# ltiao/bore

Hardware: NVIDIA B200
Metric: mlp_value_and_input_grad_evals_per_sec (higher is better)
Workload: dtype f32 MLP / f64 L-BFGS-B

## Files before the change

### bore_b200/csrc/lbfgsb.cu

```cuda
#include <float.h>
#include <math.h>
#include <stdlib.h>
#include <string.h>

#include <algorithm>
#include <cmath>

#include "common.cuh"
#include "lbfgsb_fused.h"
#include "lbfgsb_types.h"

namespace lbw {
#define LB_VARIANT 1
#include "lbfgsb_core.h"
#undef LB_VARIANT
}
namespace lbw10 {
#define LB_VARIANT 1
#define LB_MCONST 10
#include "lbfgsb_core.h"
#undef LB_MCONST
#undef LB_VARIANT
}

template <int MC> struct LbCore;
template <> struct LbCore<0> {
  using Work = lbw::LbWork;
  static __device__ __forceinline__ void carve(Work &w, double *d, int *i, int n, int m) { lbw::lb_carve(w, d, i, n, m); }
  template <class Mem>
  static __device__ __forceinline__ int advance(const LbParams &P, Work &w, LbScal &s, Mem &mem, int stage) {
    return lbw::lb_advance(P, w, s, mem, stage);
  }
};
template <> struct LbCore<10> {
  using Work = lbw10::LbWork;
  static __device__ __forceinline__ void carve(Work &w, double *d, int *i, int n, int m) { lbw10::lb_carve(w, d, i, n, m); }
  template <class Mem>
  static __device__ __forceinline__ int advance(const LbParams &P, Work &w, LbScal &s, Mem &mem, int stage) {
    return lbw10::lb_advance(P, w, s, mem, stage);
  }
};
namespace {

constexpr int SCAL_BYTES = LB_SCAL_DOUBLES * sizeof(double);
static_assert(sizeof(LbScal) <= SCAL_BYTES, "LbScal grew past its slot");

struct LbLayout {
  size_t lo, hi, nbd, cnt, work, evals, lists, xf, f, g, pend, blocks, block_stride, total;
};

__host__ __device__ inline size_t align_up(size_t a, size_t b) { return (a + b - 1) / b * b; }

inline LbLayout make_layout(int S, int n, int m) {
  LbLayout L;
  size_t o = 0;
  L.lo = o; o += align_up(n * sizeof(double), 16);
  L.hi = o; o += align_up(n * sizeof(double), 16);
  L.nbd = o; o += align_up(n * sizeof(int), 16);
  L.cnt = o; o += 16;
  L.work = o; o += 16;
  L.evals = o; o += 16;
  L.lists = o; o += align_up((size_t)2 * S * sizeof(int), 16);
  L.xf = o; o += align_up((size_t)S * n * sizeof(float), 16);
  L.f = o; o += align_up((size_t)S * sizeof(float), 16);
  L.g = o; o += align_up((size_t)S * n * sizeof(float), 16);
  L.pend = o; o += align_up((size_t)S * sizeof(int), 16);
  o = align_up(o, 256);
  L.block_stride = align_up((size_t)LB_PERSIST_DOUBLES(n, m) * sizeof(double), 128);
  L.blocks = o; o += L.block_stride * S;
  L.total = o;
  return L;
}

struct LbDev {
  LbParams P;
  int S;
  char *blocks;
  size_t block_stride;
  double *xreq;
  float *xf;
  const void *F;
  const void *G;
  int *lists;
  int *cnt;
  int *work;
  unsigned long long *evals;
  unsigned long long *bytes;
  int *pend;
};

__device__ __forceinline__ LbScal *scal_of(const LbDev &D, int sid) {
  return reinterpret_cast<LbScal *>(D.blocks + D.block_stride * sid);
}

__device__ __forceinline__ unsigned long long step_bytes(int n, int fg_size, bool was_ls,
                                                         bool heavy, int col_in, int col_out,
                                                         bool pend, bool updated) {
  unsigned long long b = 2ull * sizeof(LbScal) + (unsigned long long)fg_size * (1 + n) + 8ull * n;
  if (was_ls) b += 32ull * n;
  if (heavy && col_in > 0) b += 16ull * n * col_in + 32ull * col_in * col_in;
  b += pend ? 12ull * n : 8ull * n;
  if (heavy && pend) b += 32ull * n;
  if (updated) b += 16ull * n + 48ull * col_out + 8ull * col_out * col_out;
  return b;
}

__global__ void __launch_bounds__(128) lbfgsb_init_kernel(LbDev D, const double *__restrict__ X0) {
  const int n = D.P.n;
  const int warp = (blockIdx.x * blockDim.x + threadIdx.x) >> 5;
  const int nwarps = (gridDim.x * blockDim.x) >> 5;
  const int lane = threadIdx.x & 31;
  if (blockIdx.x == 0 && threadIdx.x == 0) {
    D.cnt[0] = D.S; D.cnt[1] = 0; D.cnt[2] = 0;
    D.work[0] = 0; D.work[1] = 0; D.work[2] = 0;
    *D.evals = 0ULL;
    *D.bytes = 0ULL;
  }
  for (int sid = warp; sid < D.S; sid += nwarps) {
    for (int i = lane; i < n; i += 32) {
      double xi = X0[(size_t)sid * n + i];
      const int nb = D.P.nbd[i];
      if (nb > 0) {
        if (nb <= 2 && xi <= D.P.lo[i]) xi = D.P.lo[i];
        else if (nb >= 2 && xi >= D.P.hi[i]) xi = D.P.hi[i];
      }
      D.xreq[(size_t)sid * n + i] = xi;
      if (D.xf) D.xf[(size_t)sid * n + i] = (float)xi;
    }
    if (lane == 0) {
      LbScal s;
      s.f = 0; s.fold = 0; s.theta = 1.0; s.gd = 0; s.gdold = 0; s.dtd = 0; s.dnorm = 0;
      s.stp = 0; s.stpmx = 0; s.sbgnrm = 0;
      s.finit = s.ginit = s.gtest = s.gx = s.gy = s.fx = s.fy = 0;
      s.stx = s.sty = s.stmin = s.stmax = s.width = s.width1 = 0;
      s.phase = LB_PH_START; s.col = 0; s.iupdat = 0; s.iter = 0; s.nit = 0;
      s.nfev = 1;
      s.ifun = 0; s.iback = 0; s.updatd = 0; s.status = -1; s.task = 0;
      s.brackt = 0; s.stage = 0; s.ls_task = LB_LS_START; s.nskip = 0; s.nintol = 0;
      s.resume = 0;
      *scal_of(D, sid) = s;
      D.lists[sid] = sid;
      if (D.pend) D.pend[sid] = 1;
    }
  }
}

__device__ __forceinline__ uint32_t smem_u32(const void *p) {
  return (uint32_t)__cvta_generic_to_shared(p);
}
__device__ __forceinline__ void mbar_init(uint64_t *bar, int count) {
  asm volatile("mbarrier.init.shared::cta.b64 [%0], %1;" ::"r"(smem_u32(bar)), "r"(count) : "memory");
}
__device__ __forceinline__ void mbar_expect_tx(uint64_t *bar, uint32_t bytes) {
  asm volatile("mbarrier.arrive.expect_tx.shared::cta.b64 _, [%0], %1;" ::"r"(smem_u32(bar)), "r"(bytes)
               : "memory");
}
__device__ __forceinline__ void mbar_wait(uint64_t *bar, uint32_t parity) {
  asm volatile(
      "{\n"
      ".reg .pred p;\n"
      "LB_WAIT:\n"
      "mbarrier.try_wait.parity.shared::cta.b64 p, [%0], %1;\n"
      "@p bra LB_DONE;\n"
      "bra LB_WAIT;\n"
      "LB_DONE:\n"
      "}\n" ::"r"(smem_u32(bar)), "r"(parity)
      : "memory");
}
__device__ __forceinline__ void bulk_g2s(void *dst_smem, const void *src, uint32_t bytes, uint64_t *bar) {
  asm volatile("cp.async.bulk.shared::cluster.global.mbarrier::complete_tx::bytes [%0], [%1], %2, [%3];"
               ::"r"(smem_u32(dst_smem)), "l"(src), "r"(bytes), "r"(smem_u32(bar))
               : "memory");
}
__device__ __forceinline__ void bulk_s2g(void *dst, const void *src_smem, uint32_t bytes) {
  asm volatile("cp.async.bulk.global.shared::cta.bulk_group [%0], [%1], %2;" ::"l"(dst),
               "r"(smem_u32(src_smem)), "r"(bytes)
               : "memory");
}
__device__ __forceinline__ void bulk_commit() { asm volatile("cp.async.bulk.commit_group;" ::: "memory"); }
__device__ __forceinline__ void bulk_wait_read() {
  asm volatile("cp.async.bulk.wait_group.read 0;" ::: "memory");
}
__device__ __forceinline__ void bulk_wait_all() {
  asm volatile("cp.async.bulk.wait_group 0;" ::: "memory");
}
__device__ __forceinline__ void bulk_prefetch_l2(const void *src, uint32_t bytes) {
  asm volatile("cp.async.bulk.prefetch.L2.global [%0], %1;" ::"l"(src), "r"(bytes) : "memory");
}
__device__ __forceinline__ void fence_async_smem() {
  asm volatile("fence.proxy.async.shared::cta;" ::: "memory");
}

constexpr int LB_NPHASE_MAX = 4;

struct BlockMem {
  bool loaded = false, is_dirty = false, vec_dirty = false, requested = false;
  __device__ bool ld_kept() { return false; }
  int nph = 0, cap = LB_NPHASE_MAX;
  uint64_t *bar = nullptr;
  uint32_t parity = 0;
  __device__ void load() {
    if (!loaded && requested) { mbar_wait(bar, parity); __syncwarp(); }
    loaded = true;
  }
  __device__ void dirty() { is_dirty = true; }
  __device__ void dirty_vec() { vec_dirty = true; }
  __device__ void phase() {
    if (nph < cap) { __syncthreads(); ++nph; }
  }
};

__host__ __device__ inline size_t lb_header_bytes(int n, int wpb) {
  return align_up(LB_FORMK_ACC * 32 * sizeof(int), 16) + 2 * align_up(n * sizeof(double), 16) +
         align_up(n * sizeof(int), 16) + align_up(2 * wpb * sizeof(uint64_t) + 2 * sizeof(int), 16);
}

template <typename FG, int MC>
__global__ void __maxnreg__(168) lbfgsb_warp_kernel(LbDev D, int round, size_t warp_bytes, int nphase, int kofn, int pf) {
  extern __shared__ __align__(128) unsigned char smem_raw[];
  const int n = D.P.n, m = D.P.m;
  const int wib = threadIdx.x >> 5, lane = threadIdx.x & 31;
  const int wpb = blockDim.x >> 5;
  const int cur = round % 3, nxt = (round + 1) % 3, clr = (round + 2) % 3;
  if (blockIdx.x == 0 && threadIdx.x == 0) { D.cnt[clr] = 0; D.work[clr] = 0; }
  const int n_active = D.cnt[cur];
  if (blockIdx.x * wpb >= n_active) return;
  const int *list_cur = D.lists + (size_t)(round & 1) * D.S;
  int *list_nxt = D.lists + (size_t)((round + 1) & 1) * D.S;
  int *qhead = D.work + cur;

  int *ftab = reinterpret_cast<int *>(smem_raw);
  double *s_lo = reinterpret_cast<double *>(smem_raw + align_up(LB_FORMK_ACC * 32 * sizeof(int), 16));
  double *s_hi = s_lo + align_up(n * sizeof(double), 16) / sizeof(double);
  int *s_nbd = reinterpret_cast<int *>(s_hi + align_up(n * sizeof(double), 16) / sizeof(double));
  uint64_t *bars = reinterpret_cast<uint64_t *>(reinterpret_cast<unsigned char *>(s_nbd) +
                                                align_up(n * sizeof(int), 16));
  uint64_t *bar = bars + 2 * wib, *bar2 = bar + 1;
  unsigned char *base = smem_raw + lb_header_bytes(n, wpb) + warp_bytes * wib;
  const uint32_t block_bytes = (uint32_t)(LB_PERSIST_DOUBLES(n, m) * sizeof(double));
  const uint32_t p1_bytes = (uint32_t)(SCAL_BYTES + 4 * LB_NV(n) * sizeof(double));
  const uint32_t p2_bytes = block_bytes - p1_bytes;

  int &kn_wait = reinterpret_cast<int *>(bars + 2 * wpb)[0];
  int &kn_done = reinterpret_cast<int *>(bars + 2 * wpb)[1];
  if (threadIdx.x == 0) { kn_wait = 0; kn_done = 0; }
  auto claim = [&]() {
    int v = 0;
    if (lane == 0) v = atomicAdd(qhead, 1);
    return __shfl_sync(0xffffffffu, v, 0);
  };
  int cur_i = claim();
  int nxt_sid = -1;
  if (lane == 0) {
    mbar_init(bar, 1);
    mbar_init(bar2, 1);
    asm volatile("fence.mbarrier_init.release.cluster;" ::: "memory");
    if (cur_i < n_active) {
      mbar_expect_tx(bar, p1_bytes);
      bulk_g2s(base, D.blocks + D.block_stride * list_cur[cur_i], p1_bytes, bar);
    }
  }
  int nxt_i = n_active;
#pragma unroll 1
  for (int o = threadIdx.x; o < LB_FORMK_ACC * 32; o += blockDim.x) ftab[o] = lbw::lb_formk_code(o, m);
#pragma unroll 1
  for (int i = threadIdx.x; i < n; i += blockDim.x) {
    s_lo[i] = D.P.lo[i];
    s_hi[i] = D.P.hi[i];
    s_nbd[i] = D.P.nbd[i];
  }
  __syncthreads();
  LbParams P = D.P;
  P.lo = s_lo; P.hi = s_hi; P.nbd = s_nbd;

  typename LbCore<MC>::Work w;
  LbCore<MC>::carve(w, reinterpret_cast<double *>(base),
                    reinterpret_cast<int *>(base + lbw::lb_work_doubles(n, m) * sizeof(double)), n, m);
  w.ftab = ftab;
  LbScal *s_smem = reinterpret_cast<LbScal *>(base);
  const FG *F = static_cast<const FG *>(D.F);
  const FG *G = static_cast<const FG *>(D.G);
  uint32_t parity = 0, parity2 = 0;
  unsigned long long my_bytes = 0, my_evals = 0;

  LbScal s;
  BlockMem mem;
  int sid = 0, col_in = 0;
  bool was_ls = false;

  auto finish = [&](int pend) {
    char *gblock = D.blocks + D.block_stride * sid;
    double *xr = D.xreq + (size_t)sid * n;
    if (mem.requested) {
      if (!mem.loaded) mbar_wait(bar2, parity2);
      parity2 ^= 1;
    }
    __syncwarp();
    my_bytes += step_bytes(n, (int)sizeof(FG), was_ls, mem.loaded, col_in, s.col, pend != 0, mem.is_dirty);
    if (pend) {
      int changed = 0;
      float *xf = D.xf ? D.xf + (size_t)sid * n : nullptr;
#pragma unroll 1
      for (int i = lane; i < n; i += 32) {
        const double xi = w.x[i];
        changed |= (xr[i] != xi);
        xr[i] = xi;
        if (xf) xf[i] = (float)xi;
      }
      if (__any_sync(0xffffffffu, changed)) s.nfev += 1;
    } else {
#pragma unroll 1
      for (int i = lane; i < n; i += 32) xr[i] = w.x[i];
    }
    if (lane == 0) *s_smem = s;
    fence_async_smem();
    __syncwarp();
    cur_i = nxt_i;
    if (lane == 0) {
      uint32_t bytes = SCAL_BYTES;
      if (pend && mem.vec_dirty) bytes += 4 * LB_NV(n) * sizeof(double);
      if (pend && mem.is_dirty) bytes = block_bytes;
      bulk_s2g(gblock, base, bytes);
      bulk_commit();
      if (pend) {
        const int pos = atomicAdd(&D.cnt[nxt], 1);
        list_nxt[pos] = sid;
        my_evals += 1;
      }
      if (D.pend) D.pend[sid] = pend;
      bulk_wait_read();
      if (cur_i < n_active) {
        mbar_expect_tx(bar, p1_bytes);
        bulk_g2s(base, D.blocks + D.block_stride * list_cur[cur_i], p1_bytes, bar);
      }
    }
    __syncwarp();
  };

#pragma unroll 1
  for (;;) {
    bool holding = false;
#pragma unroll 1
    while (cur_i < n_active) {
      sid = nxt_sid >= 0 ? nxt_sid : list_cur[cur_i];
      nxt_i = claim();
      nxt_sid = nxt_i < n_active ? list_cur[nxt_i] : -1;
      if (nxt_sid >= 0 && lane == 0) bulk_prefetch_l2(D.blocks + D.block_stride * nxt_sid, p1_bytes);
      if (nxt_sid >= 0 && pf) {
        const char *px = reinterpret_cast<const char *>(D.xreq + (size_t)nxt_sid * n);
        const char *pg = reinterpret_cast<const char *>(G + (size_t)nxt_sid * n);
        const int xb = n * (int)sizeof(double), gb = n * (int)sizeof(FG);
        const char *p = nullptr;
        if (lane < 16) { if (lane * 128 < xb) p = px + lane * 128; }
        else if (lane < 31) { if ((lane - 16) * 128 < gb) p = pg + (lane - 16) * 128; }
        else p = reinterpret_cast<const char *>(F + nxt_sid);
        if (p) asm volatile("prefetch.global.L2 [%0];" ::"l"(p));
      }
      const double *xr = D.xreq + (size_t)sid * n;
      const FG *gr = G + (size_t)sid * n;
      const double fval = (double)F[sid];
#pragma unroll 1
      for (int i = lane; i < n; i += 32) {
        w.x[i] = xr[i];
        w.g[i] = (double)gr[i];
        const int nb = s_nbd[i];
        w.iwhere[i] = nb == 0 ? -1 : ((nb == 2 && s_hi[i] - s_lo[i] <= 0.0) ? 3 : 0);
      }
      mbar_wait(bar, parity);
      parity ^= 1;
      __syncwarp();
      s = *s_smem;
      s.f = fval;
      mem = BlockMem();
      mem.cap = nphase < 0 ? 0 : nphase;
      mem.bar = bar2;
      mem.parity = parity2;
      col_in = s.col;
      was_ls = s.phase == LB_PH_LNSRCH;
      const int r = LbCore<MC>::advance(P, w, s, mem, 1);
      if (r == 2) {
        if (lane == 0) {
          mbar_expect_tx(bar2, p2_bytes);
          bulk_g2s(base + p1_bytes, D.blocks + D.block_stride * sid + p1_bytes, p2_bytes, bar2);
        }
        mem.requested = true;
        holding = true;
        break;
      }
      finish(r);
    }
    if (nphase < 0) {
      if (!holding) break;
      const int r = LbCore<MC>::advance(P, w, s, mem, 2);
      finish(r);
      continue;
    }
    if (kofn > 0) {
      if (!holding) break;
      if (lane == 0) atomicAdd(&kn_wait, 1);
      __syncwarp();
      asm volatile("bar.sync 1, %0;" ::"r"(kofn * 32) : "memory");
      if (lane == 0) atomicSub(&kn_wait, 1);
      const int r = LbCore<MC>::advance(P, w, s, mem, 2);
      finish(r);
      continue;
    }
    if (!__syncthreads_or(holding ? 1 : 0)) break;
    if (holding) {
      const int r = LbCore<MC>::advance(P, w, s, mem, 2);
#pragma unroll 1
      while (mem.nph < nphase) { __syncthreads(); ++mem.nph; }
      finish(r);
    } else {
#pragma unroll 1
      for (int k = 0; k < nphase; ++k) __syncthreads();
    }
  }
  if (lane == 0) {
    atomicAdd(D.bytes, my_bytes);
    atomicAdd(D.evals, my_evals);
    bulk_wait_all();
  }
  if (kofn > 0) {
    if (lane == 0) atomicAdd(&kn_done, 1);
#pragma unroll 1
    for (;;) {
      int done = 0, waiting = 0;
      if (lane == 0) {
        done = *reinterpret_cast<volatile int *>(&kn_done);
        waiting = *reinterpret_cast<volatile int *>(&kn_wait);
      }
      done = __shfl_sync(0xffffffffu, done, 0);
      waiting = __shfl_sync(0xffffffffu, waiting, 0);
      if (done >= wpb) break;
      if (waiting > 0) asm volatile("bar.arrive 1, %0;" ::"r"(kofn * 32) : "memory");
      __nanosleep(200);
    }
  }
}

__global__ void lbfgsb_results_kernel(LbDev D, double *x, double *fun, int *nit, int *nfev,
                                      int *status, int *task) {
  const int n = D.P.n;
  for (int sid = blockIdx.x * blockDim.x + threadIdx.x; sid < D.S; sid += gridDim.x * blockDim.x) {
    const LbScal *s = scal_of(D, sid);
    if (fun) fun[sid] = s->f;
    if (nit) nit[sid] = s->nit;
    if (nfev) nfev[sid] = s->nfev;
    if (status) status[sid] = s->status;
    if (task) task[sid] = s->task;
    if (x && x != D.xreq)
      for (int i = 0; i < n; ++i) x[(size_t)sid * n + i] = D.xreq[(size_t)sid * n + i];
  }
}

struct LbProfile {
  bool enabled = false;
  std::vector<cudaEvent_t> pool;
  double k2_ms = 0, step_ms = 0, bytes = 0, evals = 0;
  int rounds = 0, k2_launches = 0, step_launches = 0;
  int fused = 0, grid = 0, block = 0;
  double tail_ms = 0;
  cudaEvent_t get(size_t i) {
    while (pool.size() <= i) {
      cudaEvent_t e;
      cudaEventCreate(&e);
      pool.push_back(e);
    }
    return pool[i];
  }
};
LbProfile g_prof;

struct StepLaunch {
  int grid, block;
  size_t warp_bytes, smem;
};

int plan_step(int S, int n, int m, int sm_count, StepLaunch &L) {
  L.warp_bytes = align_up(lbw::lb_work_doubles(n, m) * sizeof(double) + lbw::lb_work_ints(n) * sizeof(int), 16);
  const size_t hdr = lb_header_bytes(n, 12);
  const size_t max_block = 227 * 1024, max_sm = 228 * 1024;
  BORE_CHECK(L.warp_bytes + hdr <= max_block, "lbfgsb: n=%d needs %zu B of shared memory per start", n,
             L.warp_bytes + hdr);
  int wpb = 1, best = 0;
  for (int c = 1; c <= 12; ++c) {
    if (c * L.warp_bytes + hdr > max_block) break;
    int ctas = (int)(max_sm / (c * L.warp_bytes + hdr + 1024));
    if (ctas * c > 12) ctas = 12 / c;
    if (ctas * c >= best) { best = ctas * c; wpb = c; }
  }
  {
    static int forced = -1;
    if (forced < 0) {
      const char *e = getenv("BORE_LB_WPB");
      forced = e ? atoi(e) : 0;
    }
    if (forced >= 1 && forced <= 12 && forced * L.warp_bytes + hdr <= max_block) wpb = forced;
  }
  L.block = wpb * 32;
  L.smem = hdr + wpb * L.warp_bytes;
  int per_sm = (int)(max_sm / (L.smem + 1024));
  if (per_sm * wpb > 12) per_sm = 12 / wpb;
  if (per_sm < 1) per_sm = 1;
  L.grid = sm_count * per_sm;
  const int need = (S + wpb - 1) / wpb;
  if (L.grid > need) L.grid = need;
  if (L.grid < 1) L.grid = 1;
  return 0;
}

int setup_problem(LbParams &P, double *lo_d, double *hi_d, int *nbd_d, int n, int m, const double *lo_h,
                  const double *hi_h, double ftol, double gtol, int maxiter, int maxfun, int maxls,
                  cudaStream_t stream) {
  std::vector<double> lo(n), hi(n);
  std::vector<int> nbd(n);
  int cnstnd = 0, boxed = 1;
  for (int i = 0; i < n; ++i) {
    const bool Lb = !isinf(lo_h[i]), Ub = !isinf(hi_h[i]);
    BORE_CHECK(!(Lb && Ub && lo_h[i] > hi_h[i]),
               "LBFGSB - one of the lower bounds is greater than an upper bound.");
    nbd[i] = Lb ? (Ub ? 2 : 1) : (Ub ? 3 : 0);
    lo[i] = Lb ? lo_h[i] : 0.0;
    hi[i] = Ub ? hi_h[i] : 0.0;
    if (nbd[i] != 2) boxed = 0;
    if (nbd[i] != 0) cnstnd = 1;
  }
  BORE_CUDA(cudaMemcpyAsync(lo_d, lo.data(), n * sizeof(double), cudaMemcpyHostToDevice, stream));
  BORE_CUDA(cudaMemcpyAsync(hi_d, hi.data(), n * sizeof(double), cudaMemcpyHostToDevice, stream));
  BORE_CUDA(cudaMemcpyAsync(nbd_d, nbd.data(), n * sizeof(int), cudaMemcpyHostToDevice, stream));
  BORE_CUDA(cudaStreamSynchronize(stream));
  P.n = n; P.m = m; P.maxiter = maxiter; P.maxfun = maxfun; P.maxls = maxls;
  P.cnstnd = cnstnd; P.boxed = boxed; P.ftol = ftol; P.pgtol = gtol;
  P.lo = lo_d; P.hi = hi_d; P.nbd = nbd_d;
  return 0;
}

int setup_params(LbDev &D, const LbLayout &L, char *work, int S, int n, int m, const double *lo_h,
                 const double *hi_h, double ftol, double gtol, int maxiter, int maxfun, int maxls,
                 cudaStream_t stream) {
  if (setup_problem(D.P, reinterpret_cast<double *>(work + L.lo), reinterpret_cast<double *>(work + L.hi),
                    reinterpret_cast<int *>(work + L.nbd), n, m, lo_h, hi_h, ftol, gtol, maxiter, maxfun,
                    maxls, stream))
    return -1;
  D.S = S;
  D.blocks = work + L.blocks;
  D.block_stride = L.block_stride;
  D.lists = reinterpret_cast<int *>(work + L.lists);
  D.cnt = reinterpret_cast<int *>(work + L.cnt);
  D.work = reinterpret_cast<int *>(work + L.work);
  D.evals = reinterpret_cast<unsigned long long *>(work + L.evals);
  D.bytes = D.evals + 1;
  return 0;
}

template <typename FG, int MC>
int launch_round_mc(const LbDev &D, const StepLaunch &SL, int round, int nphase, cudaStream_t stream) {
  static bool attr_done[64] = {};
  int dev = 0;
  BORE_CUDA(cudaGetDevice(&dev));
  if (dev >= 64 || !attr_done[dev]) {
    BORE_CUDA(cudaFuncSetAttribute(lbfgsb_warp_kernel<FG, MC>, cudaFuncAttributeMaxDynamicSharedMemorySize,
                                   227 * 1024));
    if (dev < 64) attr_done[dev] = true;
  }
  static int kofn = -1;
  if (kofn < 0) {
    const char *e = getenv("BORE_LB_KOFN");
    kofn = e ? atoi(e) : 0;
    if (kofn < 0) kofn = 0;
  }
  const int k_eff = (nphase == 0 && kofn > 0) ? std::min(kofn, SL.block / 32) : 0;
  static int pf = -1;
  if (pf < 0) {
    const char *e = getenv("BORE_LB_PREFETCH");
    pf = e ? atoi(e) : 1;
  }
  lbfgsb_warp_kernel<FG, MC><<<SL.grid, SL.block, SL.smem, stream>>>(D, round, SL.warp_bytes, nphase, k_eff, pf);
  BORE_CUDA(cudaGetLastError());
  return 0;
}

template <typename FG>
int launch_round(const LbDev &D, const StepLaunch &SL, int round, cudaStream_t stream) {
  static int nphase = -1;
  if (nphase < 0) {
    const char *e = getenv("BORE_LB_NPHASE");
    nphase = e ? atoi(e) : 0;
    if (nphase < -1) nphase = -1;
    if (nphase > LB_NPHASE_MAX) nphase = LB_NPHASE_MAX;
  }
  if (D.P.m == 10) return launch_round_mc<FG, 10>(D, SL, round, nphase, stream);
  return launch_round_mc<FG, 0>(D, SL, round, nphase, stream);
}

struct ExtHeader {
  LbDev D;
  int round;
  int sm_count;
};
constexpr size_t EXT_HDR = 512;
static_assert(sizeof(ExtHeader) <= EXT_HDR, "ExtHeader too large");

int check_opts(int S, int D, int m, int maxls) {
  BORE_CHECK(S >= 1, "lbfgsb: S=%d", S);
  BORE_CHECK(D >= 1 && D <= BORE_MAX_DIM, "lbfgsb: D=%d outside [1,%d]", D, BORE_MAX_DIM);
  BORE_CHECK(m >= 1 && m <= BORE_LBFGSB_MAXCOR, "lbfgsb: maxcor=%d outside [1,%d]", m,
             BORE_LBFGSB_MAXCOR);
  BORE_CHECK(maxls > 0, "maxls must be positive.");
  return 0;
}

constexpr int FUSED_MAX_STARTS = 16384, FUSED_MAX_STARTS_LARGE_N = 4096, FUSED_LARGE_N = 16;
int g_lb_mode = -1;
int lb_mode() {
  if (g_lb_mode < 0) {
    const char *e = getenv("BORE_LB_FUSED");
    const int v = e ? atoi(e) : 1;
    g_lb_mode = v == 0 ? 1 : (v == 2 ? 2 : 0);
  }
  return g_lb_mode;
}
bool use_fused(const bore_mlp *h, int S, int m, int per_model) {
  const int mode = lb_mode();
  if (mode == 1) return false;
  static const int fused_max_env = [] { const char *e = getenv("BORE_LB_FUSED_MAX"); return e ? atoi(e) : 0; }();
  const int fused_max = fused_max_env > 0 ? fused_max_env
                                          : (h->desc.dims[0] > FUSED_LARGE_N ? FUSED_MAX_STARTS_LARGE_N : FUSED_MAX_STARTS);
  if (mode == 0 && per_model == 0 && S > fused_max) return false;
  return m <= BORE_LBFGSB_MAXCOR && lbfgsb_fused_fits(h, m) != 0;
}

}

extern "C" {

size_t bore_lbfgsb_workspace_bytes(int S, int D, int m) {
  if (S < 1 || D < 1 || m < 1) return 0;
  return EXT_HDR + make_layout(S, D, m).total;
}

int bore_lbfgsb_set_mode(int mode) {
  BORE_CHECK(mode >= 0 && mode <= 2, "bore_lbfgsb_set_mode: mode %d (0 default, 1 lock-step rounds, 2 fused)", mode);
  g_lb_mode = mode;
  return 0;
}

size_t bore_lbfgsb_minimize_workspace_bytes(const bore_mlp *h, int S, int m) {
  if (!h || S < 1 || m < 1) return 0;
  const int D = h->desc.dims[0];
  if (use_fused(h, S, m, 0)) return EXT_HDR + lbfgsb_fused_workspace_bytes(D);
  return bore_lbfgsb_workspace_bytes(S, D, m);
}

static int minimize_impl(bore_mlp *h, int model, int n_models, int per_model, int transform,
                         const double *X0_dev, int S, const double *lo_host, const double *hi_host,
                         int m, double ftol, double gtol, int maxiter, int maxfun, int maxls,
                         void *work_dev, size_t work_bytes, double *x_dev, double *fun_dev,
                         int32_t *nit_dev, int32_t *nfev_dev, int32_t *status_dev, int32_t *task_dev,
                         int *rounds_out, long long *evals_out, void *stream_) {
  BORE_NVTX("bore:argmax L-BFGS-B (K2+K3 / K3f)");
  BORE_CHECK(h != nullptr, "NULL handle");
  BORE_CHECK(model >= 0 && n_models >= 1 && model + n_models <= h->n_models,
             "models [%d,%d) outside [0,%d)", model, model + n_models, h->n_models);
  const int n = h->desc.dims[0];
  if (check_opts(S, n, m, maxls)) return -1;
  BORE_CHECK(transform >= 0 && transform <= BORE_TRANSFORM_EXP, "unknown transform code %d", transform);
  BORE_CHECK(x_dev && X0_dev && work_dev, "NULL buffer");
  BORE_CUDA(cudaSetDevice(h->device));
  cudaStream_t stream = (cudaStream_t)stream_;
  if (use_fused(h, S, m, per_model)) {
    const size_t need = EXT_HDR + lbfgsb_fused_workspace_bytes(n);
    BORE_CHECK(work_bytes >= need, "lbfgsb workspace too small: %zu < %zu", work_bytes, need);
    char *work = static_cast<char *>(work_dev) + EXT_HDR;
    double *lo_d = reinterpret_cast<double *>(work + 64);
    double *hi_d = lo_d + align_up(n * sizeof(double), 16) / sizeof(double);
    int *nbd_d = reinterpret_cast<int *>(hi_d + align_up(n * sizeof(double), 16) / sizeof(double));
    LbParams P;
    if (setup_problem(P, lo_d, hi_d, nbd_d, n, m, lo_host, hi_host, ftol, gtol, maxiter, maxfun, maxls, stream))
      return -1;
    if (g_prof.enabled) cudaEventRecord(g_prof.get(0), stream);
    long long evals = 0;
    FusedLaunchInfo info;
    const int rc = launch_lbfgsb_fused(h, model, n_models, per_model, transform, X0_dev, S, P, work, x_dev,
                                       fun_dev, nit_dev, nfev_dev, status_dev, task_dev, nullptr, &info, stream);
    if (rc) return rc;
    if (g_prof.enabled) cudaEventRecord(g_prof.get(1), stream);
    BORE_CUDA(cudaMemcpyAsync(&evals, work + 8, sizeof(evals), cudaMemcpyDeviceToHost, stream));
    cudaError_t e = cudaStreamSynchronize(stream);
    if (e != cudaSuccess) { bore_set_error("lbfgsb (fused): %s", cudaGetErrorString(e)); return -2; }
    if (evals_out) *evals_out = evals;
    if (rounds_out) *rounds_out = 1;
    if (g_prof.enabled) {
      float ms = 0;
      cudaEventElapsedTime(&ms, g_prof.get(0), g_prof.get(1));
      g_prof.k2_ms = 0; g_prof.step_ms = ms; g_prof.rounds = 1;
      g_prof.k2_launches = 0; g_prof.step_launches = 1;
      g_prof.bytes = (double)S * (16.0 * n + 24.0);
      g_prof.evals = (double)evals;
      g_prof.fused = 1; g_prof.grid = info.grid; g_prof.block = info.block;
    }
    return 0;
  }
  g_prof.fused = 0;
  const LbLayout L = make_layout(S, n, m);
  BORE_CHECK(work_bytes >= EXT_HDR + L.total, "lbfgsb workspace too small: %zu < %zu", work_bytes,
             EXT_HDR + L.total);
  char *work = static_cast<char *>(work_dev) + EXT_HDR;
  LbDev D;
  if (setup_params(D, L, work, S, n, m, lo_host, hi_host, ftol, gtol, maxiter, maxfun, maxls, stream))
    return -1;
  D.xreq = x_dev;
  D.xf = reinterpret_cast<float *>(work + L.xf);
  float *F = reinterpret_cast<float *>(work + L.f);
  float *G = reinterpret_cast<float *>(work + L.g);
  D.F = F; D.G = G;
  D.pend = per_model > 0 ? reinterpret_cast<int *>(work + L.pend) : nullptr;
  StepLaunch SL;
  if (plan_step(S, n, m, h->sm_count, SL)) return -1;
  {
    const int blocks = std::min((S + 3) / 4, h->sm_count * 8);
    lbfgsb_init_kernel<<<blocks, 128, 0, stream>>>(D, X0_dev);
    BORE_CUDA(cudaGetLastError());
  }
  if (mlp_eval_prepare(h, model, n_models, true, stream)) return -1;
  const int CHUNK = 4;
  int *cnt_host = nullptr;
  BORE_CUDA(cudaMallocHost(&cnt_host, 2 * sizeof(int)));
  cudaEvent_t ev[2];
  BORE_CUDA(cudaEventCreateWithFlags(&ev[0], cudaEventDisableTiming));
  BORE_CUDA(cudaEventCreateWithFlags(&ev[1], cudaEventDisableTiming));
  int round = 0, rc = 0;
  int handover = 0, handover_max = 0;
  if (per_model == 0 && lb_mode() != 1 && m <= BORE_LBFGSB_MAXCOR && lbfgsb_fused_fits(h, m)) {
    static int hmax = -1;
    if (hmax < 0) {
      const char *e = getenv("BORE_LB_HANDOVER");
      hmax = e ? atoi(e) : 4096;
      if (hmax < 0) hmax = 0;
    }
    handover_max = hmax;
  }
  bool have_prev = false;
  int slot = 0;
  const long long max_rounds = (long long)maxfun + (long long)maxls + 8;
  for (;;) {
    for (int k = 0; k < CHUNK; ++k, ++round) {
      const int *list = D.lists + (size_t)(round & 1) * S;
      if (g_prof.enabled) cudaEventRecord(g_prof.get(3 * (size_t)round), stream);
      rc = per_model > 0
               ? launch_mlp_eval_multi(h, model, n_models, per_model, true, transform, 1, D.xf, F, G,
                                       D.pend, stream, 1)
               : launch_mlp_eval(h, model, true, transform, 1, D.xf, S, F, G, list, D.cnt + round % 3,
                                 stream, 1);
      if (rc) break;
      if (g_prof.enabled) cudaEventRecord(g_prof.get(3 * (size_t)round + 1), stream);
      rc = launch_round<float>(D, SL, round, stream);
      if (rc) break;
      if (g_prof.enabled) cudaEventRecord(g_prof.get(3 * (size_t)round + 2), stream);
    }
    if (rc) break;
    if (cudaGetLastError() != cudaSuccess) { bore_set_error("lbfgsb stepper launch failed"); rc = -2; break; }
    cudaMemcpyAsync(&cnt_host[slot], D.cnt + round % 3, sizeof(int), cudaMemcpyDeviceToHost, stream);
    cudaEventRecord(ev[slot], stream);
    if (have_prev) {
      cudaError_t e = cudaEventSynchronize(ev[slot ^ 1]);
      if (e != cudaSuccess) { bore_set_error("lbfgsb: %s", cudaGetErrorString(e)); rc = -2; break; }
      if (cnt_host[slot ^ 1] == 0) break;
      if (handover_max > 0 && cnt_host[slot ^ 1] <= handover_max) { handover = cnt_host[slot ^ 1]; break; }
    }
    have_prev = true;
    slot ^= 1;
    if (round > max_rounds) { bore_set_error("lbfgsb: exceeded %lld rounds", max_rounds); rc = -3; break; }
  }
  float tail_ms = 0.f;
  if (!rc && handover > 0) {
    FusedResume R;
    R.list = D.lists + (size_t)(round & 1) * S;
    R.count = D.cnt + round % 3;
    R.blocks = D.blocks;
    R.block_stride = D.block_stride;
    R.qhead = D.work + 3;
    R.evals = D.evals;
    if (g_prof.enabled) cudaEventRecord(g_prof.get(3 * (size_t)round), stream);
    rc = launch_lbfgsb_fused(h, model, 1, 0, transform, nullptr, handover, D.P, work, D.xreq, nullptr, nullptr,
                             nullptr, nullptr, nullptr, nullptr, nullptr, stream, &R);
    if (g_prof.enabled) cudaEventRecord(g_prof.get(3 * (size_t)round + 1), stream);
  }
  if (!rc) {
    lbfgsb_results_kernel<<<std::min((S + 127) / 128, 1024), 128, 0, stream>>>(
        D, x_dev, fun_dev, nit_dev, nfev_dev, status_dev, task_dev);
    unsigned long long evals = 0;
    cudaMemcpyAsync(&evals, D.evals, sizeof(evals), cudaMemcpyDeviceToHost, stream);
    cudaError_t e = cudaStreamSynchronize(stream);
    if (e != cudaSuccess) { bore_set_error("lbfgsb: %s", cudaGetErrorString(e)); rc = -2; }
    if (evals_out) *evals_out = (long long)evals + S;
    if (rounds_out) *rounds_out = round;
    if (g_prof.enabled && !rc) {
      unsigned long long bytes = 0;
      cudaMemcpy(&bytes, D.bytes, sizeof(bytes), cudaMemcpyDeviceToHost);
      g_prof.k2_ms = g_prof.step_ms = 0;
      for (int r = 0; r < round; ++r) {
        float a = 0, b = 0;
        cudaEventElapsedTime(&a, g_prof.get(3 * (size_t)r), g_prof.get(3 * (size_t)r + 1));
        cudaEventElapsedTime(&b, g_prof.get(3 * (size_t)r + 1), g_prof.get(3 * (size_t)r + 2));
        g_prof.k2_ms += a;
        g_prof.step_ms += b;
      }
      if (handover > 0) {
        cudaEventElapsedTime(&tail_ms, g_prof.get(3 * (size_t)round), g_prof.get(3 * (size_t)round + 1));
        g_prof.step_ms += tail_ms;
      }
      g_prof.tail_ms = tail_ms;
      g_prof.rounds = round;
      g_prof.k2_launches = g_prof.step_launches = round;
      g_prof.bytes = (double)bytes;
      g_prof.evals = (double)evals + S;
    }
  } else {
    cudaStreamSynchronize(stream);
  }
  cudaEventDestroy(ev[0]);
  cudaEventDestroy(ev[1]);
  cudaFreeHost(cnt_host);
  return rc;
}

int bore_lbfgsb_minimize(bore_mlp *h, int model, int transform, const double *X0_dev, int S,
                         const double *lo_host, const double *hi_host, int m, double ftol,
                         double gtol, int maxiter, int maxfun, int maxls, void *work_dev,
                         size_t work_bytes, double *x_dev, double *fun_dev, int32_t *nit_dev,
                         int32_t *nfev_dev, int32_t *status_dev, int32_t *task_dev, int *rounds_out,
                         long long *evals_out, void *stream_) {
  return minimize_impl(h, model, 1, 0, transform, X0_dev, S, lo_host, hi_host, m, ftol, gtol, maxiter,
                       maxfun, maxls, work_dev, work_bytes, x_dev, fun_dev, nit_dev, nfev_dev,
                       status_dev, task_dev, rounds_out, evals_out, stream_);
}

int bore_lbfgsb_minimize_multi(bore_mlp *h, int model0, int n_models, int starts_per_model,
                               int transform, const double *X0_dev, const double *lo_host,
                               const double *hi_host, int m, double ftol, double gtol, int maxiter,
                               int maxfun, int maxls, void *work_dev, size_t work_bytes,
                               double *x_dev, double *fun_dev, int32_t *nit_dev, int32_t *nfev_dev,
                               int32_t *status_dev, int32_t *task_dev, int *rounds_out,
                               long long *evals_out, void *stream_) {
  BORE_CHECK(starts_per_model >= 1 && starts_per_model <= 4096,
             "bore_lbfgsb_minimize_multi: starts_per_model=%d outside [1,4096]", starts_per_model);
  BORE_CHECK(n_models >= 1 && (long long)n_models * starts_per_model <= 0x7fffffffLL,
             "bore_lbfgsb_minimize_multi: n_models=%d", n_models);
  return minimize_impl(h, model0, n_models, starts_per_model, transform, X0_dev,
                       n_models * starts_per_model, lo_host, hi_host, m, ftol, gtol, maxiter, maxfun,
                       maxls, work_dev, work_bytes, x_dev, fun_dev, nit_dev, nfev_dev, status_dev,
                       task_dev, rounds_out, evals_out, stream_);
}

int bore_lbfgsb_profile(int enable) {
  g_prof.enabled = enable != 0;
  return 0;
}
int bore_lbfgsb_last_profile(double *out) {
  BORE_CHECK(out != nullptr, "NULL argument");
  out[0] = g_prof.k2_ms; out[1] = g_prof.step_ms; out[2] = g_prof.rounds;
  out[3] = g_prof.bytes; out[4] = g_prof.evals;
  out[5] = g_prof.fused; out[6] = g_prof.grid; out[7] = g_prof.block;
  return 0;
}

int bore_lbfgsb_init(const double *X0_dev, int S, int n, const double *lo_host,
                     const double *hi_host, int m, double ftol, double gtol, int maxiter,
                     int maxfun, int maxls, void *work_dev, size_t work_bytes, double *xreq_dev,
                     int32_t *pend_dev, int device, void *stream_) {
  if (check_opts(S, n, m, maxls)) return -1;
  BORE_CHECK(X0_dev && work_dev && xreq_dev && pend_dev, "NULL buffer");
  BORE_CHECK(bore_device_count() > 0, "no CUDA device visible -- bore_b200 has no CPU fallback");
  BORE_CUDA(cudaSetDevice(device));
  cudaStream_t stream = (cudaStream_t)stream_;
  const LbLayout L = make_layout(S, n, m);
  BORE_CHECK(work_bytes >= EXT_HDR + L.total, "lbfgsb workspace too small: %zu < %zu", work_bytes,
             EXT_HDR + L.total);
  char *work = static_cast<char *>(work_dev) + EXT_HDR;
  ExtHeader H;
  memset(&H, 0, sizeof(H));
  if (setup_params(H.D, L, work, S, n, m, lo_host, hi_host, ftol, gtol, maxiter, maxfun, maxls, stream))
    return -1;
  H.D.xreq = xreq_dev;
  H.D.xf = nullptr;
  H.D.F = nullptr; H.D.G = nullptr;
  H.D.pend = pend_dev;
  H.round = 0;
  cudaDeviceProp prop;
  BORE_CUDA(cudaGetDeviceProperties(&prop, device));
  H.sm_count = prop.multiProcessorCount;
  const int blocks = std::min((S + 3) / 4, H.sm_count * 8);
  lbfgsb_init_kernel<<<blocks, 128, 0, stream>>>(H.D, X0_dev);
  BORE_CUDA(cudaGetLastError());
  BORE_CUDA(cudaMemcpyAsync(work_dev, &H, sizeof(H), cudaMemcpyHostToDevice, stream));
  BORE_CUDA(cudaStreamSynchronize(stream));
  return 0;
}

int bore_lbfgsb_step(const void *f_dev, const void *g_dev, int fg_is_f64, int S, int n,
                     void *work_dev, double *xreq_dev, int32_t *pend_dev, int *pending_out,
                     int device, void *stream_) {
  BORE_CHECK(f_dev && g_dev && work_dev, "NULL buffer");
  BORE_CUDA(cudaSetDevice(device));
  cudaStream_t stream = (cudaStream_t)stream_;
  ExtHeader H;
  BORE_CUDA(cudaMemcpyAsync(&H, work_dev, sizeof(H), cudaMemcpyDeviceToHost, stream));
  BORE_CUDA(cudaStreamSynchronize(stream));
  BORE_CHECK(H.D.S == S && H.D.P.n == n, "lbfgsb_step: workspace was initialised for S=%d D=%d",
             H.D.S, H.D.P.n);
  H.D.F = f_dev; H.D.G = g_dev;
  H.D.xreq = xreq_dev; H.D.pend = pend_dev;
  StepLaunch SL;
  if (plan_step(S, n, H.D.P.m, H.sm_count, SL)) return -1;
  const int rc = fg_is_f64 ? launch_round<double>(H.D, SL, H.round, stream)
                           : launch_round<float>(H.D, SL, H.round, stream);
  if (rc) return rc;
  BORE_CUDA(cudaGetLastError());
  H.round += 1;
  int pending = 0;
  BORE_CUDA(cudaMemcpyAsync(&pending, H.D.cnt + H.round % 3, sizeof(int), cudaMemcpyDeviceToHost, stream));
  BORE_CUDA(cudaMemcpyAsync(work_dev, &H, sizeof(H), cudaMemcpyHostToDevice, stream));
  BORE_CUDA(cudaStreamSynchronize(stream));
  if (pending_out) *pending_out = pending;
  return 0;
}

int bore_lbfgsb_results(int S, int n, void *work_dev, double *x_dev, double *fun_dev,
                        int32_t *nit_dev, int32_t *nfev_dev, int32_t *status_dev, int32_t *task_dev,
                        int device, void *stream_) {
  BORE_CHECK(work_dev, "NULL buffer");
  BORE_CUDA(cudaSetDevice(device));
  cudaStream_t stream = (cudaStream_t)stream_;
  ExtHeader H;
  BORE_CUDA(cudaMemcpyAsync(&H, work_dev, sizeof(H), cudaMemcpyDeviceToHost, stream));
  BORE_CUDA(cudaStreamSynchronize(stream));
  BORE_CHECK(H.D.S == S && H.D.P.n == n, "lbfgsb_results: workspace was initialised for S=%d D=%d",
             H.D.S, H.D.P.n);
  lbfgsb_results_kernel<<<std::min((S + 127) / 128, 1024), 128, 0, stream>>>(
      H.D, x_dev, fun_dev, nit_dev, nfev_dev, status_dev, task_dev);
  BORE_CUDA(cudaGetLastError());
  BORE_CUDA(cudaStreamSynchronize(stream));
  return 0;
}

}
```

Measured before the change: 44.27 million.

## Stage next problem's x, g, f into shared memory via cp.async on mbarrier

Loads of x, g and f for the next L-BFGS-B problem are now issued as cp.async copies into shared memory that complete on the same mbarrier as the bulk block load. The copies start during the previous problem's finish instead of as synchronous loads at the top of the loop. The queue-claim atomic is issued early and its result consumed after advance, and the per-step x-changed comparison is replaced by a w.changed flag. This is meant to hide global load latency and atomic latency behind compute. The cost is more complex barrier accounting (count 33) and a dependence on the core setting w.changed and on w.q being usable as staging space.

```diff
diff --git a/bore_b200/csrc/lbfgsb.cu b/bore_b200/csrc/lbfgsb.cu
--- a/bore_b200/csrc/lbfgsb.cu
+++ b/bore_b200/csrc/lbfgsb.cu
@@ -190,6 +190,15 @@
 __device__ __forceinline__ void fence_async_smem() {
   asm volatile("fence.proxy.async.shared::cta;" ::: "memory");
 }
+template <int BYTES>
+__device__ __forceinline__ void cp_async_g2s(void *dst_smem, const void *src) {
+  static_assert(BYTES == 4 || BYTES == 8, "cp.async.ca copies 4, 8 or 16 bytes");
+  asm volatile("cp.async.ca.shared.global [%0], [%1], %2;" ::"r"(smem_u32(dst_smem)), "l"(src), "n"(BYTES)
+               : "memory");
+}
+__device__ __forceinline__ void cp_async_arrive(uint64_t *bar) {
+  asm volatile("cp.async.mbarrier.arrive.noinc.shared::cta.b64 [%0];" ::"r"(smem_u32(bar)) : "memory");
+}
 
 constexpr int LB_NPHASE_MAX = 4;
 
@@ -244,23 +253,20 @@
   int &kn_wait = reinterpret_cast<int *>(bars + 2 * wpb)[0];
   int &kn_done = reinterpret_cast<int *>(bars + 2 * wpb)[1];
   if (threadIdx.x == 0) { kn_wait = 0; kn_done = 0; }
-  auto claim = [&]() {
-    int v = 0;
-    if (lane == 0) v = atomicAdd(qhead, 1);
-    return __shfl_sync(0xffffffffu, v, 0);
-  };
-  int cur_i = claim();
-  int nxt_sid = -1;
+  int cur_i = 0;
+  if (lane == 0) cur_i = atomicAdd(qhead, 1);
+  cur_i = __shfl_sync(0xffffffffu, cur_i, 0);
+  int cur_sid = cur_i < n_active ? list_cur[cur_i] : -1;
   if (lane == 0) {
-    mbar_init(bar, 1);
+    mbar_init(bar, 1 + 32);
     mbar_init(bar2, 1);
     asm volatile("fence.mbarrier_init.release.cluster;" ::: "memory");
-    if (cur_i < n_active) {
+    if (cur_sid >= 0) {
       mbar_expect_tx(bar, p1_bytes);
-      bulk_g2s(base, D.blocks + D.block_stride * list_cur[cur_i], p1_bytes, bar);
-    }
-  }
-  int nxt_i = n_active;
+      bulk_g2s(base, D.blocks + D.block_stride * cur_sid, p1_bytes, bar);
+    }
+  }
+  int nxt_i = n_active, nxt_sid = -1;
 #pragma unroll 1
   for (int o = threadIdx.x; o < LB_FORMK_ACC * 32; o += blockDim.x) ftab[o] = lbw::lb_formk_code(o, m);
 #pragma unroll 1
@@ -283,12 +289,29 @@
   uint32_t parity = 0, parity2 = 0;
   unsigned long long my_bytes = 0, my_evals = 0;
 
+  const int g_off = sizeof(FG) == 4 ? LB_NV(n) : 0;
+  auto stage_light = [&](int st) {
+    const double *xr = D.xreq + (size_t)st * n;
+    const FG *gr = G + (size_t)st * n;
+    FG *gs = reinterpret_cast<FG *>(w.g) + g_off;
+#pragma unroll 1
+    for (int i = lane; i < n; i += 32) {
+      cp_async_g2s<8>(w.x + i, xr + i);
+      cp_async_g2s<sizeof(FG)>(gs + i, gr + i);
+    }
+    if (lane == 31) cp_async_g2s<sizeof(FG)>(w.q, F + st);
+    cp_async_arrive(bar);
+  };
+  if (cur_sid >= 0) stage_light(cur_sid);
+
   LbScal s;
   BlockMem mem;
   int sid = 0, col_in = 0;
   bool was_ls = false;
 
   auto finish = [&](int pend) {
+    int pos = 0;
+    if (pend && lane == 0) pos = atomicAdd(&D.cnt[nxt], 1);
     char *gblock = D.blocks + D.block_stride * sid;
     double *xr = D.xreq + (size_t)sid * n;
     if (mem.requested) {
@@ -298,16 +321,14 @@
     __syncwarp();
     my_bytes += step_bytes(n, (int)sizeof(FG), was_ls, mem.loaded, col_in, s.col, pend != 0, mem.is_dirty);
     if (pend) {
-      int changed = 0;
       float *xf = D.xf ? D.xf + (size_t)sid * n : nullptr;
 #pragma unroll 1
       for (int i = lane; i < n; i += 32) {
         const double xi = w.x[i];
-        changed |= (xr[i] != xi);
         xr[i] = xi;
         if (xf) xf[i] = (float)xi;
       }
-      if (__any_sync(0xffffffffu, changed)) s.nfev += 1;
+      if (w.changed) s.nfev += 1;
     } else {
 #pragma unroll 1
       for (int i = lane; i < n; i += 32) xr[i] = w.x[i];
@@ -316,6 +337,8 @@
     fence_async_smem();
     __syncwarp();
     cur_i = nxt_i;
+    cur_sid = nxt_sid;
+    if (cur_sid >= 0) stage_light(cur_sid);
     if (lane == 0) {
       uint32_t bytes = SCAL_BYTES;
       if (pend && mem.vec_dirty) bytes += 4 * LB_NV(n) * sizeof(double);
@@ -323,15 +346,14 @@
       bulk_s2g(gblock, base, bytes);
       bulk_commit();
       if (pend) {
-        const int pos = atomicAdd(&D.cnt[nxt], 1);
         list_nxt[pos] = sid;
         my_evals += 1;
       }
       if (D.pend) D.pend[sid] = pend;
       bulk_wait_read();
-      if (cur_i < n_active) {
+      if (cur_sid >= 0) {
         mbar_expect_tx(bar, p1_bytes);
-        bulk_g2s(base, D.blocks + D.block_stride * list_cur[cur_i], p1_bytes, bar);
+        bulk_g2s(base, D.blocks + D.block_stride * cur_sid, p1_bytes, bar);
       }
     }
     __syncwarp();
@@ -342,8 +364,39 @@
     bool holding = false;
 #pragma unroll 1
     while (cur_i < n_active) {
-      sid = nxt_sid >= 0 ? nxt_sid : list_cur[cur_i];
-      nxt_i = claim();
+      sid = cur_sid;
+      int claimed = 0;
+      if (lane == 0) claimed = atomicAdd(qhead, 1);
+#pragma unroll 1
+      for (int i = lane; i < n; i += 32) {
+        const int nb = s_nbd[i];
+        w.iwhere[i] = nb == 0 ? -1 : ((nb == 2 && s_hi[i] - s_lo[i] <= 0.0) ? 3 : 0);
+      }
+      mbar_wait(bar, parity);
+      parity ^= 1;
+      __syncwarp();
+      if (sizeof(FG) == 4) {
+        const float *gs = reinterpret_cast<const float *>(w.g) + g_off;
+#pragma unroll 1
+        for (int i0 = 0; i0 < n; i0 += 32) {
+          const int i = i0 + lane;
+          const float gi = i < n ? gs[i] : 0.f;
+          __syncwarp();
+          if (i < n) w.g[i] = (double)gi;
+        }
+        __syncwarp();
+      }
+      s = *s_smem;
+      s.f = (double)*reinterpret_cast<const FG *>(w.q);
+      __syncwarp();
+      mem = BlockMem();
+      mem.cap = nphase < 0 ? 0 : nphase;
+      mem.bar = bar2;
+      mem.parity = parity2;
+      col_in = s.col;
+      was_ls = s.phase == LB_PH_LNSRCH;
+      const int r = LbCore<MC>::advance(P, w, s, mem, 1);
+      nxt_i = __shfl_sync(0xffffffffu, claimed, 0);
       nxt_sid = nxt_i < n_active ? list_cur[nxt_i] : -1;
       if (nxt_sid >= 0 && lane == 0) bulk_prefetch_l2(D.blocks + D.block_stride * nxt_sid, p1_bytes);
       if (nxt_sid >= 0 && pf) {
@@ -356,28 +409,6 @@
         else p = reinterpret_cast<const char *>(F + nxt_sid);
         if (p) asm volatile("prefetch.global.L2 [%0];" ::"l"(p));
       }
-      const double *xr = D.xreq + (size_t)sid * n;
-      const FG *gr = G + (size_t)sid * n;
-      const double fval = (double)F[sid];
-#pragma unroll 1
-      for (int i = lane; i < n; i += 32) {
-        w.x[i] = xr[i];
-        w.g[i] = (double)gr[i];
-        const int nb = s_nbd[i];
-        w.iwhere[i] = nb == 0 ? -1 : ((nb == 2 && s_hi[i] - s_lo[i] <= 0.0) ? 3 : 0);
-      }
-      mbar_wait(bar, parity);
-      parity ^= 1;
-      __syncwarp();
-      s = *s_smem;
-      s.f = fval;
-      mem = BlockMem();
-      mem.cap = nphase < 0 ? 0 : nphase;
-      mem.bar = bar2;
-      mem.parity = parity2;
-      col_in = s.col;
-      was_ls = s.phase == LB_PH_LNSRCH;
-      const int r = LbCore<MC>::advance(P, w, s, mem, 1);
       if (r == 2) {
         if (lane == 0) {
           mbar_expect_tx(bar2, p2_bytes);
```

Result: faster. 46.67 million (median of 6 runs) (+5.4%).
